# wenjundeng/pic1dp

Hardware: AMD Instinct MI355X
Metric: particle-updates/sec (higher is better)
Workload: dtype f64

## Files before the change

pic1dp_amd/csrc/kernels_step.hip:

```cpp
#include "device_diag.hpp"
#include "device_field.hpp"
#include "device_fx.hpp"
#include "device_math.hpp"
#include "device_xchg.hpp"
#include "step_args.hpp"

#include <cstdio>
#include <type_traits>
#include <vector>

#ifndef PIC1DP_STEP_DIST
#error "compile with -DPIC1DP_STEP_DIST=0..5 (pic1dp_amd/build.py does)"
#endif

namespace pic1dp {

namespace {

#ifdef PIC1DP_TUNE_STAMPS
#define STAMP(a, k)                                                                          \
  do {                                                                                       \
    if (threadIdx.x == 0) (a).stamps[static_cast<size_t>(blockIdx.x) * 8 + (k)] = wall_clock64(); \
  } while (0)
#define STAMP_HWID(a)                                                                                             \
// ... 174 lines not shown
__device__ __forceinline__ double pred_coef_core(double v, double w, double p, double dt, const SpeciesConst &s, D &dv,
                                                 double &t2) {
  const double tmp1 = (MODE == MODE_DF_LIN) ? p : (p - w);
  t2 = dlnf0<DIST, POW2>(v, s, dv);
  return divc<POW2>(dt * tmp1 * t2 * s.Z, s.m, s.r_m, dv);
}
template <int DIST, int MODE, int POW2>
__device__ __forceinline__ double pred_coef(double v, double w, double p, double dt, const SpeciesConst &s, double &t2) {
  if constexpr (POW2 == 0) {
    if (s.fastc) {
      DivFast dv;
      const double c = pred_coef_core<DIST, MODE, POW2>(v, w, p, dt, s, dv, t2);
      if (dv.ok()) return c;
    }
  }
  DivTrue dv;
  return pred_coef_core<DIST, MODE, POW2>(v, w, p, dt, s, dv, t2);
}

struct FxTiles {
  double s0, s1;
  float mx0, mx1;
};
__device__ __forceinline__ double wave_uniform(double v) {
  const long long b = __double_as_longlong(v);
  const unsigned lo = static_cast<unsigned>(__builtin_amdgcn_readfirstlane(static_cast<int>(b)));
  const unsigned hi = static_cast<unsigned>(__builtin_amdgcn_readfirstlane(static_cast<int>(b >> 32)));
  return __longlong_as_double(static_cast<long long>((static_cast<unsigned long long>(hi) << 32) | lo));
}
__device__ __forceinline__ double fx_scale(double lim, double markers) {
  const double t = lim * markers;
  return t > 0.0 && t < 0x1p900 ? ldexp(1.0, 60 - ilogb(t)) : __builtin_inf();
}
__device__ __forceinline__ void pred_add_fx(double *p, double v, double s) {
  const double t = fma(v, s, 6755399441055744.0);
  __hip_atomic_fetch_add(reinterpret_cast<unsigned long long *>(p),
                         static_cast<unsigned long long>(__double_as_longlong(t)) - 0x4338000000000000ull, __ATOMIC_RELAXED,
                         __HIP_MEMORY_SCOPE_WORKGROUP);
}
__device__ __forceinline__ void fx_note(unsigned *slot, float seen_f) {
  for (int off = 32; off > 0; off >>= 1) seen_f = fmaxf(seen_f, __shfl_down(seen_f, off, 64));
  if ((threadIdx.x & 63) == 0) {
    const unsigned code = seen_f >= 0.0f ? __float_as_uint(seen_f) + 2u : (seen_f > -1.5f ? 1u : 0u);
    __hip_atomic_fetch_max(slot, code, __ATOMIC_RELAXED, __HIP_MEMORY_SCOPE_WORKGROUP);
  }
}

template <int DIST, int MODE, int POW2, int NM>
__device__ __forceinline__ double pred_one(const One &n, double p, int ix, double wl, const double *sAB, double *sP,
                                           const StepArgsDev &a, FxTiles &fx) {
  constexpr int nm = NM, np1 = 1 + 2 * NM;
  const double xh = fma(a.dt_half, n.v, n.x);
  const double sh = xh * a.snx;
  const double fh = floor(sh);
  int ih = static_cast<int>(fh);
  const double wr = sh - fh, wh = 1.0 - wr;
  ih = ih < 0 ? ih + a.g.nx : ih;
  ih = ih > a.g.nx ? ih - a.g.nx : ih;
  if (static_cast<unsigned>(ih) > static_cast<unsigned>(a.g.nx)) {
    ih = ih % a.g.nx;
    if (ih < 0) ih += a.g.nx;
  }
  double *cl = sP + __mul24(ih, np1), *cr = cl + np1;
  double t2 = 0.0;
  auto slow = [&](int k, double vl, double vr) {
    const int nx = a.g.nx;
    const int gl_c = ih >= nx ? ih - nx : ih;
    int gr_c = ih + 1;
    gr_c = gr_c >= nx ? gr_c - nx : gr_c;
    gr_c = gr_c >= nx ? gr_c - nx : gr_c;
    if (vl != 0.0) glb_add(a.pred + static_cast<size_t>(k) * nx + gl_c, vl);
    if (vr != 0.0) glb_add(a.pred + static_cast<size_t>(k) * nx + gr_c, vr);
    if (vl != 0.0 || vr != 0.0)
      __hip_atomic_fetch_add(reinterpret_cast<unsigned long long *>(a.fxb + 2), 1ull, __ATOMIC_RELAXED, __HIP_MEMORY_SCOPE_AGENT);
  };
  if constexpr (MODE == MODE_FULLF) {
    const double aq = fabs(p);
    const bool fixed = aq * fx.s0 <= a.fx_cap;
    fx.mx0 = fmaxf(fx.mx0, (fixed || fx.s0 > 0x1p1000) ? static_cast<float>(aq) : -1.0f);
    if (fixed) {
      pred_add_fx(cl, wh * p, fx.s0);
      pred_add_fx(cr, wr * p, fx.s0);
    } else {
      slow(0, wh * p, wr * p);
    }
  } else {
    const double tmp1 = (MODE == MODE_DF_LIN) ? p : (p - n.w);
    if constexpr (POW2 == 0) {
      if (a.s.fastc) {
        DivFast dv;
        t2 = dlnf0<DIST, POW2>(n.v, a.s, dv);
        if (!dv.ok()) {
          DivTrue dt;
          t2 = dlnf0<DIST, POW2>(n.v, a.s, dt);
        }
      } else {
        DivTrue dt;
        t2 = dlnf0<DIST, POW2>(n.v, a.s, dt);
      }
    } else {
      DivTrue dt;
      t2 = dlnf0<DIST, POW2>(n.v, a.s, dt);
    }
    const double c = tmp1 * t2 * a.pred_k;
    const double aq = fabs(n.w), ac = fabs(c);
    const bool ok0 = aq * fx.s0 <= a.fx_cap, ok1 = 2.0 * ac * fx.s1 <= a.fx_cap;
    fx.mx0 = fmaxf(fx.mx0, (ok0 || fx.s0 > 0x1p1000) ? static_cast<float>(aq) : -1.0f);
    fx.mx1 = fmaxf(fx.mx1, (ok1 || fx.s1 > 0x1p1000) ? static_cast<float>(ac) : -1.0f);
    const bool fixed = ok0 && ok1;
    if (fixed) {
      pred_add_fx(cl, wh * n.w, fx.s0);
      pred_add_fx(cr, wr * n.w, fx.s0);
    } else {
      slow(0, wh * n.w, wr * n.w);
    }
    const double *gl = sAB + __mul24(ix, 2 * nm), *gr = gl + 2 * nm;
    const double wlr = 1.0 - wl;
#pragma unroll
    for (int m = 0; m < nm; ++m) {
      const double2 tl = *reinterpret_cast<const double2 *>(gl + 2 * m), tr = *reinterpret_cast<const double2 *>(gr + 2 * m);
      const double A = fma(tr.x, wlr, tl.x * wl), B = fma(tr.y, wlr, tl.y * wl);
      const double cA = c * A, cB = c * B;
      if (fixed) {
        pred_add_fx(cl + 1 + m, wh * cA, fx.s1);
        pred_add_fx(cr + 1 + m, wr * cA, fx.s1);
        pred_add_fx(cl + 1 + nm + m, wh * cB, fx.s1);
        pred_add_fx(cr + 1 + nm + m, wr * cB, fx.s1);
      } else {
        slow(1 + m, wh * cA, wr * cA);
        slow(1 + nm + m, wh * cB, wr * cB);
      }
    }
  }
  return t2;
}

constexpr int FUSED_CHAIN_W = 8;
struct TabCells {
  double *ab;
  __device__ __forceinline__ void put(int c, double a, double b) const { ab[2 * c] = a, ab[2 * c + 1] = b; }
  __device__ __forceinline__ void get(int c, double &a, double &b) const { a = ab[2 * c], b = ab[2 * c + 1]; }
};
struct TabTiles {
  double *sa, *sb;
  __device__ __forceinline__ void put(int c, double a, double b) const { sa[c] = a, sb[c] = b; }
  __device__ __forceinline__ void get(int c, double &a, double &b) const { a = sa[c], b = sb[c]; }
};
template <bool TILE_EH, class TAB>
__device__ __forceinline__ void fused_solve(const FusedSolve &fs, const TAB &tab, double *sE0, double *sX, double *sSc,
                                            double &re_h, double &im_h, unsigned long long *stamps = nullptr) {
  (void)stamps;
  const FieldArgs &f = fs.f;
  const int nx = f.nx;
  double *sMode = sSc, *sScr = sSc + 8, *sPart = sSc + 24;
  const bool lead = blockIdx.x == 0;
  double *sPc = sE0, *sPs = sX;
  for (int ix = threadIdx.x; ix < nx; ix += blockDim.x) {
    double c2 = 0.0;
    for (int sp = 0; sp < f.nspecies; ++sp) {
      const double *r = f.rho_sp + static_cast<size_t>(sp) * nx + ix;
      double c1 = *r;
      for (int g = 1; g < f.rho_copies; ++g) c1 = c1 + r[static_cast<size_t>(g) * f.rho_stride];
      c2 = c2 + c1 * f.Z[sp];
    }
    const double cd = chargeden_from(f, c2);
    if (lead) {
      f.charge[ix] = c2;
      f.chargeden[ix] = cd;
    }
    const double tr = f.fre[ix], ti = f.fim[ix];
    tab.put(ix, 2.0 * tr, 2.0 * ti);
    if (ix == 0) tab.put(nx, 2.0 * tr, 2.0 * ti);
    sPc[ix] = tr * cd;
    sPs[ix] = ti * cd;
  }
  if (lead) {
    for (int64_t i = threadIdx.x; i < fs.zero_rho_n; i += blockDim.x) fs.zero_rho[i] = 0.0;
    for (int i = threadIdx.x; i < 8 * PRED_SUM_COPIES; i += blockDim.x) fs.zero_pred[i] = 0.0;
  }
  __syncthreads();
  STAMP_SOLVE(stamps, 2);
  const double ginv = f.grad_inv[0];
  {
    const double acc = lean_forward_sums<FUSED_CHAIN_W>(f, sPc, sPs, sPart, [&]() {
      const int k = static_cast<int>(threadIdx.x) - (static_cast<int>(blockDim.x) - 64);
      if (k >= 0 && k < 6) {
        double a = 0.0;
        static_assert(PRED_SUM_COPIES % 8 == 0, "eight copies in flight at a time");
        for (int c0 = 0; c0 < PRED_SUM_COPIES; c0 += 8) {
          double t[8];
#pragma unroll
          for (int c = 0; c < 8; ++c) t[c] = fs.pred_in[(c0 + c) * 8 + k];
#pragma unroll
          for (int c = 0; c < 8; ++c) a = (c0 + c == 0) ? t[0] : a + t[c];
        }
        sMode[2 + k] = a;
      }
    });
    if (threadIdx.x < 2) mode_store(f, sMode, 1, 0, threadIdx.x == 0, acc, ginv, lead);
  }
  __syncthreads();
  STAMP_SOLVE(stamps, 3);
  const double re = sMode[0], im = sMode[1];
  double ac, as;
  pred_forward_sums(f, fs.pt, sMode + 2, re, im, ac, as);
  STAMP_SOLVE(stamps, 4);
  im_h = mode_scale(f, true, ac, ginv);
  re_h = mode_scale(f, false, as, ginv);
  if (lead && threadIdx.x == 0) {
    fs.mode_h[0] = re_h;
    fs.mode_h[1] = im_h;
  }
  double e2 = 0.0;
  for (int ix = threadIdx.x; ix < nx; ix += blockDim.x) {
    double tA, tB;
    tab.get(ix, tA, tB);
    const double tr = 0.5 * tA, ti = 0.5 * tB;
    const double e = inverse_one_mode(tr, ti, re, im), eh = inverse_one_mode(tr, ti, re_h, im_h);
    sE0[ix] = e;
    if constexpr (TILE_EH) sX[ix] = eh;
    if (ix == 0) {
      sE0[nx] = e;
      if constexpr (TILE_EH) sX[nx] = eh;
    }
    e2 += e * e;
    if (lead) {
      f.E[ix] = e;
      fs.E_h[ix] = eh;
    }
  }
  if (lead && f.history) field_energy_store(e2, sScr, f.lx, f.dnx, f.history);
}

constexpr int PRIV_THREADS = STEP_PRIVATE_THREADS;
template <int DIST, int MODE, int POW2>
__device__ __forceinline__ double pred_one_private(const One &n, double p, int ix, double wl, const double *sAB, double *sS,
                                                   const StepArgsDev &a) {
  constexpr int stride = PRIV_THREADS;
  const int nx = a.g.nx;
  double t2 = 0.0, cA = 0.0, cB = 0.0;
  if constexpr (MODE != MODE_FULLF) {
    const double tmp1 = (MODE == MODE_DF_LIN) ? p : (p - n.w);
    if constexpr (POW2 == 0) {
      if (a.s.fastc) {
        DivFast dv;
        t2 = dlnf0<DIST, POW2>(n.v, a.s, dv);
        if (!dv.ok()) {
          DivTrue dt;
          t2 = dlnf0<DIST, POW2>(n.v, a.s, dt);
        }
      } else {
        DivTrue dt;
        t2 = dlnf0<DIST, POW2>(n.v, a.s, dt);
      }
    } else {
      DivTrue dt;
      t2 = dlnf0<DIST, POW2>(n.v, a.s, dt);
    }
    const double c = tmp1 * t2 * (a.pred_k * a.s.Z);
    const double *gl = sAB + 2 * ix;
    const double2 tl = *reinterpret_cast<const double2 *>(gl), tr = *reinterpret_cast<const double2 *>(gl + 2);
    const double wlr = 1.0 - wl;
    cA = c * fma(tr.x, wlr, tl.x * wl);
    cB = c * fma(tr.y, wlr, tl.y * wl);
  }
  const double xh = fma(a.dt_half, n.v, n.x);
  const double sh = xh * a.snx;
  const double fh = floor(sh);
  int ih = static_cast<int>(fh);
  const double wr = sh - fh, wh = 1.0 - wr;
  ih = ih < 0 ? ih + nx : ih;
  ih = ih >= nx ? ih - nx : ih;
  if (static_cast<unsigned>(ih) >= static_cast<unsigned>(nx)) {
    ih = ih % nx;
    if (ih < 0) ih += nx;
  }
  const double *hl = sAB + 2 * ih;
  const double2 ul = *reinterpret_cast<const double2 *>(hl), ur = *reinterpret_cast<const double2 *>(hl + 2);
  const double Ah = fma(ur.x, wr, ul.x * wh), Bh = fma(ur.y, wr, ul.y * wh);
  const double q = a.s.Z * (MODE == MODE_FULLF ? p : n.w);
  lds_add(sS, q * Ah);
  lds_add(sS + 3 * stride, q * Bh);
  if constexpr (MODE != MODE_FULLF) {
    lds_add(sS + stride, cA * Ah);
    lds_add(sS + 2 * stride, cB * Ah);
    lds_add(sS + 4 * stride, cA * Bh);
    lds_add(sS + 5 * stride, cB * Bh);
  }
  return t2;
}


template <int DIST, int MODE, int POW2, int NM>
__device__ __forceinline__ double priv_sums(const One &n, double p, int ix, double wl, const double *sAB, double *sS,
                                            const StepArgsDev &a) {
  return pred_one_private<DIST, MODE, POW2>(n, p, ix, wl, sAB, sS, a);
}

template <bool NT>
__device__ __forceinline__ bool chunk_plain(int64_t j, const StepArgsDev &a) {
  if constexpr (!NT) return false;
  return __builtin_amdgcn_readfirstlane(static_cast<int>(j >> 6)) < a.plain_chunks;
}
template <bool NT, bool HAS_W>
__device__ __forceinline__ void ld_marker_rows(bool plain, const double2 *x2, const double2 *v2, const double2 *w2, const double2 *p2,
                                               int64_t o, double2 &X, double2 &V, double2 &W, double2 &P) {
  if (NT && plain) {
    X = ld2t<false>(x2 + o), V = ld2t<false>(v2 + o), P = ld2t<false>(p2 + o);
    if constexpr (HAS_W) W = ld2t<false>(w2 + o);
  } else {
    X = ld2t<NT>(x2 + o), V = ld2t<NT>(v2 + o), P = ld2t<NT>(p2 + o);
    if constexpr (HAS_W) W = ld2t<NT>(w2 + o);
  }
}
template <bool NT, bool PUSH_V, bool HAS_W>
__device__ __forceinline__ void st_marker_rows(bool plain, double2 *x2, double2 *v2, double2 *w2, int64_t o, const One &n0, const One &n1) {
  if (NT && plain) {
    st2t<false>(x2 + o, n0.x, n1.x);
    if constexpr (PUSH_V) st2t<false>(v2 + o, n0.v, n1.v);
    if constexpr (HAS_W) st2t<false>(w2 + o, n0.w, n1.w);
  } else {
    st2t<NT>(x2 + o, n0.x, n1.x);
    if constexpr (PUSH_V) st2t<NT>(v2 + o, n0.v, n1.v);
    if constexpr (HAS_W) st2t<NT>(w2 + o, n0.w, n1.w);
  }
}

template <int DIST, int MODE, int POW2, bool NT, int T2, int NM, bool PRIV = false, bool FUSED = false>
__global__ void __launch_bounds__(1024) PIC1DP_SIX_WAVES k_step_one(const StepArgsDev a) {
  static_assert(!FUSED || PRIV, "the fused solve serves the six-sum prediction");
  constexpr int NS = 6, PT = PRIV_THREADS;
  static_assert(!PRIV || NM == 1, "six sums: one kept mode");
  extern __shared__ __attribute__((aligned(16))) char smem[];
  STAMP(a, 0);
  STAMP_HWID(a);
  exp_table_init();
  const int nx = a.g.nx;
  constexpr int nm = NM, np1 = 1 + 2 * NM;
  const int ne = (nx + 2) & ~1;
  double *sE0 = reinterpret_cast<double *>(smem);
  double *sEh = sE0 + ne;
  double *sAB = sEh + ne;
  double *sR0 = sAB + static_cast<size_t>(nx + 1) * 2 * nm;
  double *sP = sR0 + ((nx + 2) & ~1);
  if constexpr (!FUSED) {
    for (int i = threadIdx.x; i < nx; i += blockDim.x) {
      sE0[i] = a.E0[i];
      sEh[i] = a.Eh[i];
    }
  }
  if constexpr (!FUSED) {
    for (int i = threadIdx.x; i < nm * (nx + 1); i += blockDim.x) {
      const int m = i / (nx + 1), c = i - m * (nx + 1), cs = c < nx ? c : 0;
      sAB[c * 2 * nm + 2 * m] = a.tabA[m * nx + cs];
      sAB[c * 2 * nm + 2 * m + 1] = a.tabB[m * nx + cs];
    }
  }
  zero_rho(sR0, a.g);
  if constexpr (FUSED) {
    double re_h, im_h;
#ifdef PIC1DP_TUNE_STAMPS
    fused_solve<true>(a.fused, TabCells{sAB}, sE0, sEh, sP, re_h, im_h, a.stamps);
#else
    fused_solve<true>(a.fused, TabCells{sAB}, sE0, sEh, sP, re_h, im_h);
#endif
    __syncthreads();
  } else if (threadIdx.x == 0) {
    sE0[nx] = a.E0[0];
    sEh[nx] = a.Eh[0];
  }
  unsigned *sDraw = reinterpret_cast<unsigned *>(PRIV ? sP + NS * PT : sP + np1 * (nx + 2));
  FxTiles fx{};
  fx.mx0 = fx.mx1 = -2.0f;
  double fxb_start0 = 0.0, fxb_start1 = 0.0;
  if constexpr (PRIV) {
    for (int k = 0; k < NS; ++k) sP[k * PT + threadIdx.x] = 0.0;
  } else {
    if (threadIdx.x == 0) {
      sP[0] = __hip_atomic_load(a.fxb, __ATOMIC_RELAXED, __HIP_MEMORY_SCOPE_AGENT);
      sP[1] = __hip_atomic_load(a.fxb + 1, __ATOMIC_RELAXED, __HIP_MEMORY_SCOPE_AGENT);
    }
    __syncthreads();
    fxb_start0 = wave_uniform(sP[0]);
    fxb_start1 = wave_uniform(sP[1]);
    fx.s0 = wave_uniform(fx_scale(16.0 * fxb_start0, a.fx_markers));
    fx.s1 = wave_uniform(fx_scale(32.0 * fxb_start1, a.fx_markers));
    __syncthreads();
    for (int i = threadIdx.x; i < np1 * (nx + 2); i += blockDim.x) sP[i] = 0.0;
  }
  if (threadIdx.x == 0) sDraw[0] = sDraw[1] = sDraw[2] = 0u;
  __syncthreads();
  STAMP(a, 1);
  double *sR = sR0;
  constexpr bool HAS_W = (MODE != MODE_FULLF);
  constexpr bool PUSH_V = (MODE != MODE_DF_LIN);
  constexpr bool CARRY_IN = (T2 == 2) && HAS_W;
  constexpr bool CARRY_OUT = (T2 != 0) && HAS_W;
  const int64_t npair = a.np >> 1;
  const int64_t stride = static_cast<int64_t>(gridDim.x) * blockDim.x;
  double2 *x2 = reinterpret_cast<double2 *>(a.x);
  double2 *v2 = reinterpret_cast<double2 *>(a.v);
  double2 *w2 = reinterpret_cast<double2 *>(a.w);
  const double2 *p2 = reinterpret_cast<const double2 *>(a.p);
  double2 *t2 = reinterpret_cast<double2 *>(a.t2);
  const int64_t first = static_cast<int64_t>(blockIdx.x) * blockDim.x;
  int dealt = first < npair ? static_cast<int>((npair - first + stride - 1) / stride) : 0;
  int drawn_total = 0;
  if (a.dyn_tail > 0) {
    const int drawn_rows = (dealt * a.dyn_tail) >> 4;
    dealt -= drawn_rows;
    drawn_total = drawn_rows * static_cast<int>(blockDim.x >> 6);
  }
  int64_t j = first + threadIdx.x;
  for (int k = 0;; ++k, j += stride) {
    if (k >= dealt) {
      int c = 0;
      if ((threadIdx.x & 63) == 0) c = static_cast<int>(__hip_atomic_fetch_add(sDraw, 1u, __ATOMIC_RELAXED, __HIP_MEMORY_SCOPE_WORKGROUP));
      c = __builtin_amdgcn_readfirstlane(c);
      if (c >= drawn_total) break;
      const int waves = static_cast<int>(blockDim.x >> 6);
      j = first + static_cast<int64_t>(dealt + c / waves) * stride + (c % waves) * 64 + (threadIdx.x & 63);
    }
    if (j >= npair) continue;
    const int64_t o = tidx2(j);
    const bool plain = chunk_plain<NT>(j, a);
    double2 X, V, P, W = make_double2(0.0, 0.0), T = make_double2(0.0, 0.0);
    ld_marker_rows<NT, HAS_W>(plain, x2, v2, w2, p2, o, X, V, W, P);
    if constexpr (CARRY_IN) T = ld2t<NT>(t2 + j);
    int i0, i1;
    double l0, l1;
    const One n0 = step_full_one<DIST, MODE, POW2, CARRY_IN>(X.x, V.x, W.x, P.x, sE0, sEh, sR, a, T.x, &i0, &l0);
    double u0, u1;
    if constexpr (PRIV)
      u0 = priv_sums<DIST, MODE, POW2, NM>(n0, P.x, i0, l0, sAB, sP + threadIdx.x, a);
    else
      u0 = pred_one<DIST, MODE, POW2, NM>(n0, P.x, i0, l0, sAB, sP, a, fx);
    PAIR_FENCE();
    const One n1 = step_full_one<DIST, MODE, POW2, CARRY_IN>(X.y, V.y, W.y, P.y, sE0, sEh, sR, a, T.y, &i1, &l1);
    if constexpr (PRIV)
      u1 = priv_sums<DIST, MODE, POW2, NM>(n1, P.y, i1, l1, sAB, sP + threadIdx.x, a);
    else
      u1 = pred_one<DIST, MODE, POW2, NM>(n1, P.y, i1, l1, sAB, sP, a, fx);
    st_marker_rows<NT, PUSH_V, HAS_W>(plain, x2, v2, w2, o, n0, n1);
    if constexpr (CARRY_OUT) st2t<NT>(t2 + j, u0, u1);
  }
  if ((a.np & 1) && blockIdx.x == 0 && threadIdx.x == 0) {
    const int64_t i = tidx(a.np - 1);
    const double w = HAS_W ? a.w[i] : 0.0, p = a.p[i];
    int ic;
    double lc;
    const One n = step_full_one<DIST, MODE, POW2, CARRY_IN>(a.x[i], a.v[i], w, p, sE0, sEh, sR, a,
                                                            CARRY_IN ? a.t2[a.np - 1] : 0.0, &ic, &lc);
    a.x[i] = n.x;
    if constexpr (PUSH_V) a.v[i] = n.v;
    if constexpr (HAS_W) a.w[i] = n.w;
    double u;
    if constexpr (PRIV)
      u = priv_sums<DIST, MODE, POW2, NM>(n, p, ic, lc, sAB, sP + threadIdx.x, a);
    else
      u = pred_one<DIST, MODE, POW2, NM>(n, p, ic, lc, sAB, sP, a, fx);
    if constexpr (CARRY_OUT) a.t2[a.np - 1] = u;
  }
  STAMP_LOOP(a, 2);
  if constexpr (!PRIV) {
    fx_note(sDraw + 1, fx.mx0);
    fx_note(sDraw + 2, fx.mx1);
  }
  __syncthreads();
  STAMP_LOOP(a, 3);
  flush_rho(sR0, a.rho, a.g);
  STAMP_LOOP(a, 4);
  if constexpr (PRIV) {
    const int wave = threadIdx.x >> 6, lane = threadIdx.x & 63;
    if (wave < 6) {
      const double *s = sP + wave * PRIV_THREADS + lane;
      double t = 0.0;
#pragma unroll
      for (int j = 0; j < PRIV_THREADS / 64; ++j) t += s[64 * j];
      for (int off = 32; off > 0; off >>= 1) t += __shfl_down(t, off, 64);
      if (lane == 0) glb_add(a.pred + (blockIdx.x % PRED_SUM_COPIES) * 8 + wave, t);
    }
    STAMP(a, 5);
    if constexpr (!FUSED)
      if (a.tail.mode) step_tail(a.tail, reinterpret_cast<double *>(smem));
    return;
  }
  if (threadIdx.x < 2 * np1) {
    const int g = threadIdx.x / np1, k = threadIdx.x - g * np1;
    const int to = (nx + g) % nx;
    if (g == 0 || to != 0 || nx > 1)
      __hip_atomic_fetch_add(reinterpret_cast<unsigned long long *>(&sP[to * np1 + k]),
                             static_cast<unsigned long long>(__double_as_longlong(sP[(nx + g) * np1 + k])), __ATOMIC_RELAXED,
                             __HIP_MEMORY_SCOPE_WORKGROUP);
  }
  __syncthreads();
  {
    const double q0 = 1.0 / fx.s0, q1 = 1.0 / fx.s1;
    const int rot = static_cast<int>((static_cast<long long>(blockIdx.x) * nx) / gridDim.x);
    for (int i = threadIdx.x; i < np1 * nx; i += blockDim.x) {
      const int k = i / nx;
      int c = i - k * nx + rot;
      if (c >= nx) c -= nx;
      const long long fixed = __double_as_longlong(sP[c * np1 + k]);
      if (fixed != 0) glb_add(&a.pred[static_cast<size_t>(k) * nx + c], static_cast<double>(fixed) * (k == 0 ? q0 : q1));
    }
  }
  if (threadIdx.x == 0) {
    fx_raise(a.fxb, sDraw[1], fxb_start0);
    fx_raise(a.fxb + 1, sDraw[2], fxb_start1);
  }
  STAMP(a, 5);
}

struct PredSums {
  double k0c = 0.0, k1c = 0.0, k2c = 0.0, k0s = 0.0, k1s = 0.0, k2s = 0.0;
};

template <int DIST, int MODE, int POW2>
__device__ __forceinline__ double pred_one_sums(const One &n, double p, int ix, double wl, const double *sA,
                                                const double *sB, PredSums &k, const StepArgsDev &a) {
  double t2 = 0.0;
  double cA = 0.0, cB = 0.0;
  if constexpr (MODE != MODE_FULLF) {
    const double c = a.s.Z * pred_coef<DIST, MODE, POW2>(n.v, n.w, p, a.dt_half, a.s, t2);
    PAIR_FENCE();
    double A = sA[ix] * wl;
    A = A + sA[ix + 1] * (1.0 - wl);
    double B = sB[ix] * wl;
    B = B + sB[ix + 1] * (1.0 - wl);
    cA = c * A, cB = c * B;
  }
  double xh = n.x + a.dt_half * n.v;
  xh = wrap(xh, a.g.lx);
  int ih;
  double wh;
  locate(xh, a.g, ih, wh);
  double Ah = sA[ih] * wh;
  Ah = Ah + sA[ih + 1] * (1.0 - wh);
  double Bh = sB[ih] * wh;
  Bh = Bh + sB[ih + 1] * (1.0 - wh);
  const double q = a.s.Z * (MODE == MODE_FULLF ? p : n.w);
  k.k0c += q * Ah;
  k.k0s += q * Bh;
  if constexpr (MODE != MODE_FULLF) {
    k.k1c += cA * Ah;
    k.k2c += cB * Ah;
    k.k1s += cA * Bh;
    k.k2s += cB * Bh;
  }
  return t2;
}

#ifdef PIC1DP_SUMS_WAVES
#define PIC1DP_SUMS_ATTR __attribute__((amdgpu_waves_per_eu(PIC1DP_SUMS_WAVES)))
#else
#define PIC1DP_SUMS_ATTR
#endif
template <int DIST, int MODE, int POW2, bool NT, int T2, bool FUSED = false>
__global__ void __launch_bounds__(1024) PIC1DP_SUMS_ATTR k_step_sums(const StepArgsDev a) {
  extern __shared__ __attribute__((aligned(16))) char smem[];
  STAMP(a, 0);
  STAMP_HWID(a);
  exp_table_init();
  const int nx = a.g.nx;
  const int ne = (nx + 2) & ~1;
  double *sE0 = reinterpret_cast<double *>(smem);
  double *sA = sE0 + ne;
  double *sB = sA + ne;
  double *sR0 = sB + ne;
  double *sScr = sR0 + ((nx + 2) & ~1);
  unsigned *sDraw = reinterpret_cast<unsigned *>(sScr);
  if constexpr (!FUSED) {
    for (int i = threadIdx.x; i < nx; i += blockDim.x) {
      sE0[i] = a.E0[i];
      sA[i] = a.tabA[i];
      sB[i] = a.tabB[i];
    }
    if (threadIdx.x == 0) {
      sE0[nx] = a.E0[0];
      sA[nx] = a.tabA[0];
      sB[nx] = a.tabB[0];
    }
  }
  double re_h, im_h;
  if constexpr (FUSED) {
    fused_solve<false>(a.fused, TabTiles{sA, sB}, sE0, sR0, sScr, re_h, im_h);
  } else {
    re_h = *a.eh_re;
    im_h = *a.eh_im;
  }
  zero_rho(sR0, a.g);
  if (threadIdx.x == 0) *sDraw = 0u;
  __syncthreads();
  STAMP(a, 1);
  const ModeField sEh{sA, sB, re_h, im_h};
  double *sR = sR0;
  constexpr bool HAS_W = (MODE != MODE_FULLF);
  constexpr bool PUSH_V = (MODE != MODE_DF_LIN);
  constexpr bool CARRY_IN = (T2 == 2) && HAS_W;
  constexpr bool CARRY_OUT = (T2 != 0) && HAS_W;
  PredSums ks;
  const int64_t npair = a.np >> 1;
  const int64_t stride = static_cast<int64_t>(gridDim.x) * blockDim.x;
  double2 *x2 = reinterpret_cast<double2 *>(a.x);
  double2 *v2 = reinterpret_cast<double2 *>(a.v);
  double2 *w2 = reinterpret_cast<double2 *>(a.w);
  const double2 *p2 = reinterpret_cast<const double2 *>(a.p);
  double2 *t2 = reinterpret_cast<double2 *>(a.t2);
  const int64_t first = static_cast<int64_t>(blockIdx.x) * blockDim.x;
  int dealt = first < npair ? static_cast<int>((npair - first + stride - 1) / stride) : 0;
  int drawn_total = 0;
  if (a.dyn_tail > 0) {
    const int drawn_rows = (dealt * a.dyn_tail) >> 4;
    dealt -= drawn_rows;
    drawn_total = drawn_rows * static_cast<int>(blockDim.x >> 6);
  }
  int64_t j = first + threadIdx.x;
  for (int k = 0;; ++k, j += stride) {
    if (k >= dealt) {
      int c = 0;
      if ((threadIdx.x & 63) == 0) c = static_cast<int>(__hip_atomic_fetch_add(sDraw, 1u, __ATOMIC_RELAXED, __HIP_MEMORY_SCOPE_WORKGROUP));
      c = __builtin_amdgcn_readfirstlane(c);
      if (c >= drawn_total) break;
      const int waves = static_cast<int>(blockDim.x >> 6);
      j = first + static_cast<int64_t>(dealt + c / waves) * stride + (c % waves) * 64 + (threadIdx.x & 63);
    }
    if (j >= npair) continue;
    const int64_t o = tidx2(j);
    const bool plain = chunk_plain<NT>(j, a);
    double2 X, V, P, W = make_double2(0.0, 0.0), T = make_double2(0.0, 0.0);
    ld_marker_rows<NT, HAS_W>(plain, x2, v2, w2, p2, o, X, V, W, P);
    if constexpr (CARRY_IN) T = ld2t<NT>(t2 + j);
    int i0, i1;
    double l0, l1;
    const One n0 = step_full_one<DIST, MODE, POW2, CARRY_IN>(X.x, V.x, W.x, P.x, sE0, sEh, sR, a, T.x, &i0, &l0);
    PAIR_FENCE();
    const double u0 = pred_one_sums<DIST, MODE, POW2>(n0, P.x, i0, l0, sA, sB, ks, a);
    PAIR_FENCE();
    const One n1 = step_full_one<DIST, MODE, POW2, CARRY_IN>(X.y, V.y, W.y, P.y, sE0, sEh, sR, a, T.y, &i1, &l1);
    PAIR_FENCE();
    const double u1 = pred_one_sums<DIST, MODE, POW2>(n1, P.y, i1, l1, sA, sB, ks, a);
    st_marker_rows<NT, PUSH_V, HAS_W>(plain, x2, v2, w2, o, n0, n1);
    if constexpr (CARRY_OUT) st2t<NT>(t2 + j, u0, u1);
  }
  if ((a.np & 1) && blockIdx.x == 0 && threadIdx.x == 0) {
    const int64_t i = tidx(a.np - 1);
    const double w = HAS_W ? a.w[i] : 0.0, p = a.p[i];
    int ic;
    double lc;
    const One n = step_full_one<DIST, MODE, POW2, CARRY_IN>(a.x[i], a.v[i], w, p, sE0, sEh, sR, a,
                                                            CARRY_IN ? a.t2[a.np - 1] : 0.0, &ic, &lc);
    a.x[i] = n.x;
    if constexpr (PUSH_V) a.v[i] = n.v;
    if constexpr (HAS_W) a.w[i] = n.w;
    const double u = pred_one_sums<DIST, MODE, POW2>(n, p, ic, lc, sA, sB, ks, a);
    if constexpr (CARRY_OUT) a.t2[a.np - 1] = u;
  }
  STAMP_LOOP(a, 2);
  __syncthreads();
  STAMP_LOOP(a, 3);
  flush_rho(sR0, a.rho, a.g);
  STAMP_LOOP(a, 4);
  const double mine[6] = {ks.k0c, ks.k1c, ks.k2c, ks.k0s, ks.k1s, ks.k2s};
  block_sum6_add(mine, sScr, a.pred + (blockIdx.x % PRED_SUM_COPIES) * 8);
  STAMP(a, 5);
  if constexpr (!FUSED)
    if (a.tail.mode) step_tail(a.tail, reinterpret_cast<double *>(smem));
}

#ifdef PIC1DP_TUNE_STAMPS
constexpr size_t kStampGrid = 16384;
struct StampState {
  unsigned long long *dev = nullptr;
  long launches = 0, at = -1;
  int blocks = 0, threads = 0;
};
StampState &stamp_state() {
  static StampState s;
  return s;
}
hipError_t stamp_hook(StepArgsDev &d, const LaunchCfg &lc, hipStream_t st) {
  StampState &s = stamp_state();
  if (!s.dev) {
    hipError_t e = hipMalloc(&s.dev, sizeof(unsigned long long) * 8 * kStampGrid);
    if (e != hipSuccess) return e;
    if (const char *a = tuning_env("PIC1DP_STAMP_AT")) s.at = std::atol(a);
  }
  if (s.launches == s.at + 1 && s.at >= 0) {
    hipError_t e = hipStreamSynchronize(st);
    if (e != hipSuccess) return e;
    std::vector<unsigned long long> h(static_cast<size_t>(8) * s.blocks);
    e = hipMemcpy(h.data(), s.dev, sizeof(unsigned long long) * h.size(), hipMemcpyDeviceToHost);
    if (e != hipSuccess) return e;
    if (const char *fn = tuning_env("PIC1DP_STAMP_FILE")) {
      if (FILE *f = std::fopen(fn, "w")) {
        std::fprintf(f, "# blocks %d threads %d\n", s.blocks, s.threads);
        for (int b = 0; b < s.blocks; ++b) {
          for (int k = 0; k < 7; ++k) std::fprintf(f, "%llu ", h[static_cast<size_t>(b) * 8 + k]);
          std::fprintf(f, "\n");
        }
        std::fclose(f);
      }
    }
  }
  s.launches++;
  s.blocks = lc.blocks;
  s.threads = lc.threads;
  d.stamps = s.dev;
  return static_cast<size_t>(lc.blocks) <= kStampGrid ? hipSuccess : hipErrorInvalidValue;
}
#endif

template <typename K>
hipError_t launch_step_kernel(K kern, const StepArgsDev &d0, const LaunchCfg &lc, hipStream_t st) {
#ifdef PIC1DP_TUNE_STAMPS
  StepArgsDev d = d0;
  if (hipError_t e = stamp_hook(d, lc, st); e != hipSuccess) return e;
#else
  const StepArgsDev &d = d0;
#endif
  return launch_kernel(kern, dim3(lc.blocks), dim3(lc.threads), lc.lds, st, d);
}

#ifdef PIC1DP_TUNING
template <int DIST>
constexpr bool kCarryBuilt = true;
template <int DIST>
constexpr bool kNoCarryBuilt = true;
#else
template <int DIST>
constexpr bool kCarryBuilt = DIST == 2 || DIST == 3;
template <int DIST>
constexpr bool kNoCarryBuilt = !(DIST == 2 || DIST == 3);
#endif

template <int DIST, class F>
hipError_t with_nt_t2(bool nt, int t2m, F &&f) {
  auto by_t2 = [&](auto NT) -> hipError_t {
    if constexpr (kCarryBuilt<DIST>) {
      if (t2m == 2) return f(NT, std::integral_constant<int, 2>{});
      if (t2m == 1) return f(NT, std::integral_constant<int, 1>{});
    }
    if (t2m != 0) return hipErrorInvalidValue;
    if constexpr (kNoCarryBuilt<DIST>) return f(NT, std::integral_constant<int, 0>{});
    return hipErrorInvalidValue;
  };
  return nt ? by_t2(std::true_type{}) : by_t2(std::false_type{});
}

static_assert(PRED_MAX_MODES == 2 || PRED_MAX_MODES == 3, "k_step_one is instantiated for one and two (three) kept modes");
static_assert(PRIV_THREADS == STEP_PRIVATE_THREADS, "slot stride of k_step_one<PRIV> = its workgroup size");

template <int DIST, int MODE, int POW2, bool CARRY = false>
hipError_t launch_step_dmp(const StepArgs &a, bool full, const LaunchCfg &lc, hipStream_t st) {
  const StepArgsDev &d = a.d;
  const bool one_pass = full && d.pred;
  const int t2m = d.t2 ? d.t2_mode : 0;
  if (one_pass && a.family == StepFamily::PrivateSums) {
    if (d.fused.on)
      return with_nt_t2<DIST>(d.nt, t2m, [&](auto NT, auto T2) {
        return launch_step_kernel(k_step_one<DIST, MODE, POW2, NT, T2, 1, true, true>, d, lc, st);
      });
    return with_nt_t2<DIST>(d.nt, t2m, [&](auto NT, auto T2) {
      return launch_step_kernel(k_step_one<DIST, MODE, POW2, NT, T2, 1, true>, d, lc, st);
    });
  }
  if (one_pass && a.family == StepFamily::Sums) {
    if (d.fused.on)
      return with_nt_t2<DIST>(d.nt, t2m, [&](auto NT, auto T2) {
        return launch_step_kernel(k_step_sums<DIST, MODE, POW2, NT, T2, true>, d, lc, st);
      });
    return with_nt_t2<DIST>(d.nt, t2m, [&](auto NT, auto T2) {
      return launch_step_kernel(k_step_sums<DIST, MODE, POW2, NT, T2>, d, lc, st);
    });
  }
  if (d.fx.acc) {
    if (d.pred || d.dist_out) return hipErrorInvalidValue;
    if (d.nt)
      return full ? launch_step_kernel(k_step_full<DIST, MODE, POW2, true, CARRY, false, false, true>, d, lc, st)
                  : launch_step_kernel(k_step_half<DIST, MODE, POW2, true, CARRY, true>, d, lc, st);
    return full ? launch_step_kernel(k_step_full<DIST, MODE, POW2, false, CARRY, false, false, true>, d, lc, st)
                : launch_step_kernel(k_step_half<DIST, MODE, POW2, false, CARRY, true>, d, lc, st);
  }
  if (one_pass) {
    auto tiles = [&](auto NM) {
      return with_nt_t2<DIST>(d.nt, t2m, [&](auto NT, auto T2) {
        return launch_step_kernel(k_step_one<DIST, MODE, POW2, NT, T2, NM>, d, lc, st);
      });
    };
    if (d.pred_nm == 1) return tiles(std::integral_constant<int, 1>{});
    if (d.pred_nm == 2) return tiles(std::integral_constant<int, 2>{});
    if constexpr (PRED_MAX_MODES >= 3)
      if (d.pred_nm == 3) return tiles(std::integral_constant<int, 3>{});
    return hipErrorInvalidValue;
  }
  if (full && d.dist_out) {
    if (d.diag_fx)
      return d.nt ? launch_step_kernel(k_step_full<DIST, MODE, POW2, true, CARRY, true, true>, d, lc, st)
                  : launch_step_kernel(k_step_full<DIST, MODE, POW2, false, CARRY, true, true>, d, lc, st);
    return d.nt ? launch_step_kernel(k_step_full<DIST, MODE, POW2, true, CARRY, true>, d, lc, st)
                : launch_step_kernel(k_step_full<DIST, MODE, POW2, false, CARRY, true>, d, lc, st);
  }
  if (d.nt)
    return full ? launch_step_kernel(k_step_full<DIST, MODE, POW2, true, CARRY, false>, d, lc, st)
                : launch_step_kernel(k_step_half<DIST, MODE, POW2, true, CARRY>, d, lc, st);
  return full ? launch_step_kernel(k_step_full<DIST, MODE, POW2, false, CARRY, false>, d, lc, st)
              : launch_step_kernel(k_step_half<DIST, MODE, POW2, false, CARRY>, d, lc, st);
}

template <int DIST>
hipError_t launch_step_d(const StepArgs &a, bool full, const LaunchCfg &lc, hipStream_t st) {
  const StepArgsDev &d = a.d;
  const bool pow2 = d.s.pow2 != 0;
  if (!a.deltaf) {
    if constexpr (DIST == 0)
      return pow2 ? launch_step_dmp<0, MODE_FULLF, 1>(a, full, lc, st)
                  : launch_step_dmp<0, MODE_FULLF, 0>(a, full, lc, st);
    return hipErrorInvalidValue;
  }
  const bool carry = !pow2 && d.t2 != nullptr && (DIST == 2 || DIST == 3);
  if (a.linear) {
    if constexpr (DIST == 2 || DIST == 3)
      if (carry) return launch_step_dmp<DIST, MODE_DF_LIN, 0, true>(a, full, lc, st);
    return pow2 ? launch_step_dmp<DIST, MODE_DF_LIN, 1>(a, full, lc, st)
                : launch_step_dmp<DIST, MODE_DF_LIN, 0>(a, full, lc, st);
  }
  if (d.s.unit) return launch_step_dmp<DIST, MODE_DF_NL, 2>(a, full, lc, st);
  if constexpr (DIST == 2 || DIST == 3)
    if (carry) return launch_step_dmp<DIST, MODE_DF_NL, 0, true>(a, full, lc, st);
  return pow2 ? launch_step_dmp<DIST, MODE_DF_NL, 1>(a, full, lc, st)
              : launch_step_dmp<DIST, MODE_DF_NL, 0>(a, full, lc, st);
}

}

template <>
hipError_t launch_step_dist<PIC1DP_STEP_DIST>(const StepArgs &a, bool full, const LaunchCfg &lc, hipStream_t st) {
  return launch_step_d<PIC1DP_STEP_DIST>(a, full, lc, st);
}

}
```

Before: 215.7 billion.

## Restructure particle loop into wave-uniform chunks with optional row prefetch

Replaces the per-thread grid-stride loop with wave-granular chunk scheduling. Chunk base addresses are computed as scalar (readfirstlane) values plus a per-lane 16-byte offset, which should reduce per-lane 64-bit address arithmetic and VGPR use. Adds an optional software prefetch of the next chunk's X/V (or all four) rows, controlled by PIC1DP_PREFETCH_ROWS. That option defaults to 0, so by default only the addressing and scheduling restructure takes effect. Prefetching would raise register pressure in exchange for hiding load latency.

After: 215.6 billion, median of 3. No clear change (-0.1%).

```diff
diff --git a/pic1dp_amd/csrc/kernels_step.hip b/pic1dp_amd/csrc/kernels_step.hip
--- a/pic1dp_amd/csrc/kernels_step.hip
+++ b/pic1dp_amd/csrc/kernels_step.hip
@@ -500,29 +500,95 @@
   if constexpr (!NT) return false;
   return __builtin_amdgcn_readfirstlane(static_cast<int>(j >> 6)) < a.plain_chunks;
 }
-template <bool NT, bool HAS_W>
-__device__ __forceinline__ void ld_marker_rows(bool plain, const double2 *x2, const double2 *v2, const double2 *w2, const double2 *p2,
-                                               int64_t o, double2 &X, double2 &V, double2 &W, double2 &P) {
+
+struct WaveChunks {
+  int64_t first, stride;
+  int wave, waves;
+  int dealt, drawn_total;
+  int k;
+};
+__device__ __forceinline__ WaveChunks wave_chunks(int64_t npair, int dyn_tail) {
+  WaveChunks w;
+  w.first = static_cast<int64_t>(blockIdx.x) * blockDim.x;
+  w.stride = static_cast<int64_t>(gridDim.x) * blockDim.x;
+  w.wave = __builtin_amdgcn_readfirstlane(static_cast<int>(threadIdx.x >> 6));
+  w.waves = static_cast<int>(blockDim.x >> 6);
+  w.dealt = w.first < npair ? static_cast<int>((npair - w.first + w.stride - 1) / w.stride) : 0;
+  w.drawn_total = 0;
+  if (dyn_tail > 0) {
+    const int drawn_rows = (w.dealt * dyn_tail) >> 4;
+    w.dealt -= drawn_rows;
+    w.drawn_total = drawn_rows * w.waves;
+  }
+  w.k = 0;
+  return w;
+}
+__device__ __forceinline__ int64_t next_chunk(WaveChunks &w, int64_t npair, unsigned *sDraw) {
+  for (;;) {
+    int64_t j0;
+    if (w.k < w.dealt) {
+      j0 = w.first + static_cast<int64_t>(w.k) * w.stride + w.wave * 64;
+      ++w.k;
+    } else {
+      int c = 0;
+      if ((threadIdx.x & 63) == 0) c = static_cast<int>(__hip_atomic_fetch_add(sDraw, 1u, __ATOMIC_RELAXED, __HIP_MEMORY_SCOPE_WORKGROUP));
+      c = __builtin_amdgcn_readfirstlane(c);
+      if (c >= w.drawn_total) return -1;
+      j0 = w.first + static_cast<int64_t>(w.dealt + c / w.waves) * w.stride + (c % w.waves) * 64;
+    }
+    if (j0 < npair) return j0;
+  }
+}
+__device__ __forceinline__ bool chunk_lane(int64_t j0, int64_t npair, unsigned lane16) {
+  const int64_t left = npair - j0;
+  return lane16 < (left < 64 ? static_cast<unsigned>(left) << 4 : 1024u);
+}
+template <class T>
+__device__ __forceinline__ T *chunk_row(T *array, int64_t ob, unsigned lane16) {
+  const unsigned long long b = reinterpret_cast<unsigned long long>(array) + static_cast<unsigned long long>(ob);
+  const unsigned lo = static_cast<unsigned>(__builtin_amdgcn_readfirstlane(static_cast<int>(b)));
+  const unsigned hi = static_cast<unsigned>(__builtin_amdgcn_readfirstlane(static_cast<int>(b >> 32)));
+  using G = __attribute__((address_space(1))) T;
+  return (T *)reinterpret_cast<G *>(((static_cast<unsigned long long>(hi) << 32) | lo) + lane16);
+}
+template <bool NT, bool HAS_W, int R0, int R1>
+__device__ __forceinline__ void ld_chunk_rows(bool plain, const StepArgsDev &a, int64_t ob, unsigned lane16, double2 &X, double2 &V,
+                                              double2 &W, double2 &P) {
+  const double2 *x2 = chunk_row(reinterpret_cast<const double2 *>(a.x), ob, lane16);
+  const double2 *v2 = chunk_row(reinterpret_cast<const double2 *>(a.v), ob, lane16);
+  const double2 *p2 = chunk_row(reinterpret_cast<const double2 *>(a.p), ob, lane16);
+  const double2 *w2 = chunk_row(reinterpret_cast<const double2 *>(a.w), ob, lane16);
   if (NT && plain) {
-    X = ld2t<false>(x2 + o), V = ld2t<false>(v2 + o), P = ld2t<false>(p2 + o);
-    if constexpr (HAS_W) W = ld2t<false>(w2 + o);
+    if constexpr (R0 <= 0 && 0 < R1) X = ld2t<false>(x2);
+    if constexpr (R0 <= 1 && 1 < R1) V = ld2t<false>(v2);
+    if constexpr (R0 <= 2 && 2 < R1) P = ld2t<false>(p2);
+    if constexpr (HAS_W && R0 <= 3 && 3 < R1) W = ld2t<false>(w2);
   } else {
-    X = ld2t<NT>(x2 + o), V = ld2t<NT>(v2 + o), P = ld2t<NT>(p2 + o);
-    if constexpr (HAS_W) W = ld2t<NT>(w2 + o);
+    if constexpr (R0 <= 0 && 0 < R1) X = ld2t<NT>(x2);
+    if constexpr (R0 <= 1 && 1 < R1) V = ld2t<NT>(v2);
+    if constexpr (R0 <= 2 && 2 < R1) P = ld2t<NT>(p2);
+    if constexpr (HAS_W && R0 <= 3 && 3 < R1) W = ld2t<NT>(w2);
   }
 }
 template <bool NT, bool PUSH_V, bool HAS_W>
-__device__ __forceinline__ void st_marker_rows(bool plain, double2 *x2, double2 *v2, double2 *w2, int64_t o, const One &n0, const One &n1) {
+__device__ __forceinline__ void st_chunk_rows(bool plain, const StepArgsDev &a, int64_t ob, unsigned lane16, const One &n0, const One &n1) {
+  double2 *x2 = chunk_row(reinterpret_cast<double2 *>(a.x), ob, lane16);
+  double2 *v2 = chunk_row(reinterpret_cast<double2 *>(a.v), ob, lane16);
+  double2 *w2 = chunk_row(reinterpret_cast<double2 *>(a.w), ob, lane16);
   if (NT && plain) {
-    st2t<false>(x2 + o, n0.x, n1.x);
-    if constexpr (PUSH_V) st2t<false>(v2 + o, n0.v, n1.v);
-    if constexpr (HAS_W) st2t<false>(w2 + o, n0.w, n1.w);
+    st2t<false>(x2, n0.x, n1.x);
+    if constexpr (PUSH_V) st2t<false>(v2, n0.v, n1.v);
+    if constexpr (HAS_W) st2t<false>(w2, n0.w, n1.w);
   } else {
-    st2t<NT>(x2 + o, n0.x, n1.x);
-    if constexpr (PUSH_V) st2t<NT>(v2 + o, n0.v, n1.v);
-    if constexpr (HAS_W) st2t<NT>(w2 + o, n0.w, n1.w);
-  }
-}
+    st2t<NT>(x2, n0.x, n1.x);
+    if constexpr (PUSH_V) st2t<NT>(v2, n0.v, n1.v);
+    if constexpr (HAS_W) st2t<NT>(w2, n0.w, n1.w);
+  }
+}
+#ifndef PIC1DP_PREFETCH_ROWS
+#define PIC1DP_PREFETCH_ROWS 0
+#endif
+static_assert(PIC1DP_PREFETCH_ROWS == 0 || PIC1DP_PREFETCH_ROWS == 2 || PIC1DP_PREFETCH_ROWS == 4, "none, X and V, or all four rows");
 
 template <int DIST, int MODE, int POW2, bool NT, int T2, int NM, bool PRIV = false, bool FUSED = false>
 __global__ void __launch_bounds__(1024) PIC1DP_SIX_WAVES k_step_one(const StepArgsDev a) {
@@ -595,52 +661,53 @@
   constexpr bool CARRY_IN = (T2 == 2) && HAS_W;
   constexpr bool CARRY_OUT = (T2 != 0) && HAS_W;
   const int64_t npair = a.np >> 1;
-  const int64_t stride = static_cast<int64_t>(gridDim.x) * blockDim.x;
-  double2 *x2 = reinterpret_cast<double2 *>(a.x);
-  double2 *v2 = reinterpret_cast<double2 *>(a.v);
-  double2 *w2 = reinterpret_cast<double2 *>(a.w);
-  const double2 *p2 = reinterpret_cast<const double2 *>(a.p);
   double2 *t2 = reinterpret_cast<double2 *>(a.t2);
-  const int64_t first = static_cast<int64_t>(blockIdx.x) * blockDim.x;
-  int dealt = first < npair ? static_cast<int>((npair - first + stride - 1) / stride) : 0;
-  int drawn_total = 0;
-  if (a.dyn_tail > 0) {
-    const int drawn_rows = (dealt * a.dyn_tail) >> 4;
-    dealt -= drawn_rows;
-    drawn_total = drawn_rows * static_cast<int>(blockDim.x >> 6);
-  }
-  int64_t j = first + threadIdx.x;
-  for (int k = 0;; ++k, j += stride) {
-    if (k >= dealt) {
-      int c = 0;
-      if ((threadIdx.x & 63) == 0) c = static_cast<int>(__hip_atomic_fetch_add(sDraw, 1u, __ATOMIC_RELAXED, __HIP_MEMORY_SCOPE_WORKGROUP));
-      c = __builtin_amdgcn_readfirstlane(c);
-      if (c >= drawn_total) break;
-      const int waves = static_cast<int>(blockDim.x >> 6);
-      j = first + static_cast<int64_t>(dealt + c / waves) * stride + (c % waves) * 64 + (threadIdx.x & 63);
-    }
-    if (j >= npair) continue;
-    const int64_t o = tidx2(j);
-    const bool plain = chunk_plain<NT>(j, a);
-    double2 X, V, P, W = make_double2(0.0, 0.0), T = make_double2(0.0, 0.0);
-    ld_marker_rows<NT, HAS_W>(plain, x2, v2, w2, p2, o, X, V, W, P);
-    if constexpr (CARRY_IN) T = ld2t<NT>(t2 + j);
-    int i0, i1;
-    double l0, l1;
-    const One n0 = step_full_one<DIST, MODE, POW2, CARRY_IN>(X.x, V.x, W.x, P.x, sE0, sEh, sR, a, T.x, &i0, &l0);
-    double u0, u1;
-    if constexpr (PRIV)
-      u0 = priv_sums<DIST, MODE, POW2, NM>(n0, P.x, i0, l0, sAB, sP + threadIdx.x, a);
-    else
-      u0 = pred_one<DIST, MODE, POW2, NM>(n0, P.x, i0, l0, sAB, sP, a, fx);
-    PAIR_FENCE();
-    const One n1 = step_full_one<DIST, MODE, POW2, CARRY_IN>(X.y, V.y, W.y, P.y, sE0, sEh, sR, a, T.y, &i1, &l1);
-    if constexpr (PRIV)
-      u1 = priv_sums<DIST, MODE, POW2, NM>(n1, P.y, i1, l1, sAB, sP + threadIdx.x, a);
-    else
-      u1 = pred_one<DIST, MODE, POW2, NM>(n1, P.y, i1, l1, sAB, sP, a, fx);
-    st_marker_rows<NT, PUSH_V, HAS_W>(plain, x2, v2, w2, o, n0, n1);
-    if constexpr (CARRY_OUT) st2t<NT>(t2 + j, u0, u1);
+  constexpr int PF = PIC1DP_PREFETCH_ROWS;
+  const unsigned lane16 = (threadIdx.x & 63u) << 4;
+  WaveChunks wc = wave_chunks(npair, a.dyn_tail);
+  double2 X = make_double2(0.0, 0.0), V = X, P = X, W = X, Xn = X, Vn = X, Pn = X, Wn = X;
+  int64_t j0 = next_chunk(wc, npair, sDraw);
+  if constexpr (PF > 0)
+    if (j0 >= 0 && chunk_lane(j0, npair, lane16))
+      ld_chunk_rows<NT, HAS_W, 0, PF>(chunk_plain<NT>(j0, a), a, tidx2(j0) << 4, lane16, Xn, Vn, Wn, Pn);
+  while (j0 >= 0) {
+    const int64_t ob = tidx2(j0) << 4;
+    const bool plain = chunk_plain<NT>(j0, a);
+    const bool mine = chunk_lane(j0, npair, lane16);
+    int64_t jn = -1;
+    double2 T = make_double2(0.0, 0.0);
+    if constexpr (PF > 0) {
+      X = Xn, V = Vn;
+      if constexpr (PF > 2) P = Pn, W = Wn;
+      jn = next_chunk(wc, npair, sDraw);
+    }
+    if (mine) {
+      ld_chunk_rows<NT, HAS_W, PF, 4>(plain, a, ob, lane16, X, V, W, P);
+      if constexpr (CARRY_IN) T = ld2t<NT>(chunk_row(t2, j0 << 4, lane16));
+    }
+    if constexpr (PF > 0)
+      if (jn >= 0 && chunk_lane(jn, npair, lane16))
+        ld_chunk_rows<NT, HAS_W, 0, PF>(chunk_plain<NT>(jn, a), a, tidx2(jn) << 4, lane16, Xn, Vn, Wn, Pn);
+    if (mine) {
+      int i0, i1;
+      double l0, l1;
+      const One n0 = step_full_one<DIST, MODE, POW2, CARRY_IN>(X.x, V.x, W.x, P.x, sE0, sEh, sR, a, T.x, &i0, &l0);
+      double u0, u1;
+      if constexpr (PRIV)
+        u0 = priv_sums<DIST, MODE, POW2, NM>(n0, P.x, i0, l0, sAB, sP + threadIdx.x, a);
+      else
+        u0 = pred_one<DIST, MODE, POW2, NM>(n0, P.x, i0, l0, sAB, sP, a, fx);
+      PAIR_FENCE();
+      const One n1 = step_full_one<DIST, MODE, POW2, CARRY_IN>(X.y, V.y, W.y, P.y, sE0, sEh, sR, a, T.y, &i1, &l1);
+      if constexpr (PRIV)
+        u1 = priv_sums<DIST, MODE, POW2, NM>(n1, P.y, i1, l1, sAB, sP + threadIdx.x, a);
+      else
+        u1 = pred_one<DIST, MODE, POW2, NM>(n1, P.y, i1, l1, sAB, sP, a, fx);
+      st_chunk_rows<NT, PUSH_V, HAS_W>(plain, a, ob, lane16, n0, n1);
+      if constexpr (CARRY_OUT) st2t<NT>(chunk_row(t2, j0 << 4, lane16), u0, u1);
+    }
+    if constexpr (PF == 0) jn = next_chunk(wc, npair, sDraw);
+    j0 = jn;
   }
   if ((a.np & 1) && blockIdx.x == 0 && threadIdx.x == 0) {
     const int64_t i = tidx(a.np - 1);
@@ -799,47 +866,48 @@
   constexpr bool CARRY_OUT = (T2 != 0) && HAS_W;
   PredSums ks;
   const int64_t npair = a.np >> 1;
-  const int64_t stride = static_cast<int64_t>(gridDim.x) * blockDim.x;
-  double2 *x2 = reinterpret_cast<double2 *>(a.x);
-  double2 *v2 = reinterpret_cast<double2 *>(a.v);
-  double2 *w2 = reinterpret_cast<double2 *>(a.w);
-  const double2 *p2 = reinterpret_cast<const double2 *>(a.p);
   double2 *t2 = reinterpret_cast<double2 *>(a.t2);
-  const int64_t first = static_cast<int64_t>(blockIdx.x) * blockDim.x;
-  int dealt = first < npair ? static_cast<int>((npair - first + stride - 1) / stride) : 0;
-  int drawn_total = 0;
-  if (a.dyn_tail > 0) {
-    const int drawn_rows = (dealt * a.dyn_tail) >> 4;
-    dealt -= drawn_rows;
-    drawn_total = drawn_rows * static_cast<int>(blockDim.x >> 6);
-  }
-  int64_t j = first + threadIdx.x;
-  for (int k = 0;; ++k, j += stride) {
-    if (k >= dealt) {
-      int c = 0;
-      if ((threadIdx.x & 63) == 0) c = static_cast<int>(__hip_atomic_fetch_add(sDraw, 1u, __ATOMIC_RELAXED, __HIP_MEMORY_SCOPE_WORKGROUP));
-      c = __builtin_amdgcn_readfirstlane(c);
-      if (c >= drawn_total) break;
-      const int waves = static_cast<int>(blockDim.x >> 6);
-      j = first + static_cast<int64_t>(dealt + c / waves) * stride + (c % waves) * 64 + (threadIdx.x & 63);
-    }
-    if (j >= npair) continue;
-    const int64_t o = tidx2(j);
-    const bool plain = chunk_plain<NT>(j, a);
-    double2 X, V, P, W = make_double2(0.0, 0.0), T = make_double2(0.0, 0.0);
-    ld_marker_rows<NT, HAS_W>(plain, x2, v2, w2, p2, o, X, V, W, P);
-    if constexpr (CARRY_IN) T = ld2t<NT>(t2 + j);
-    int i0, i1;
-    double l0, l1;
-    const One n0 = step_full_one<DIST, MODE, POW2, CARRY_IN>(X.x, V.x, W.x, P.x, sE0, sEh, sR, a, T.x, &i0, &l0);
-    PAIR_FENCE();
-    const double u0 = pred_one_sums<DIST, MODE, POW2>(n0, P.x, i0, l0, sA, sB, ks, a);
-    PAIR_FENCE();
-    const One n1 = step_full_one<DIST, MODE, POW2, CARRY_IN>(X.y, V.y, W.y, P.y, sE0, sEh, sR, a, T.y, &i1, &l1);
-    PAIR_FENCE();
-    const double u1 = pred_one_sums<DIST, MODE, POW2>(n1, P.y, i1, l1, sA, sB, ks, a);
-    st_marker_rows<NT, PUSH_V, HAS_W>(plain, x2, v2, w2, o, n0, n1);
-    if constexpr (CARRY_OUT) st2t<NT>(t2 + j, u0, u1);
+  constexpr int PF = PIC1DP_PREFETCH_ROWS;
+  const unsigned lane16 = (threadIdx.x & 63u) << 4;
+  WaveChunks wc = wave_chunks(npair, a.dyn_tail);
+  double2 X = make_double2(0.0, 0.0), V = X, P = X, W = X, Xn = X, Vn = X, Pn = X, Wn = X;
+  int64_t j0 = next_chunk(wc, npair, sDraw);
+  if constexpr (PF > 0)
+    if (j0 >= 0 && chunk_lane(j0, npair, lane16))
+      ld_chunk_rows<NT, HAS_W, 0, PF>(chunk_plain<NT>(j0, a), a, tidx2(j0) << 4, lane16, Xn, Vn, Wn, Pn);
+  while (j0 >= 0) {
+    const int64_t ob = tidx2(j0) << 4;
+    const bool plain = chunk_plain<NT>(j0, a);
+    const bool mine = chunk_lane(j0, npair, lane16);
+    int64_t jn = -1;
+    double2 T = make_double2(0.0, 0.0);
+    if constexpr (PF > 0) {
+      X = Xn, V = Vn;
+      if constexpr (PF > 2) P = Pn, W = Wn;
+      jn = next_chunk(wc, npair, sDraw);
+    }
+    if (mine) {
+      ld_chunk_rows<NT, HAS_W, PF, 4>(plain, a, ob, lane16, X, V, W, P);
+      if constexpr (CARRY_IN) T = ld2t<NT>(chunk_row(t2, j0 << 4, lane16));
+    }
+    if constexpr (PF > 0)
+      if (jn >= 0 && chunk_lane(jn, npair, lane16))
+        ld_chunk_rows<NT, HAS_W, 0, PF>(chunk_plain<NT>(jn, a), a, tidx2(jn) << 4, lane16, Xn, Vn, Wn, Pn);
+    if (mine) {
+      int i0, i1;
+      double l0, l1;
+      const One n0 = step_full_one<DIST, MODE, POW2, CARRY_IN>(X.x, V.x, W.x, P.x, sE0, sEh, sR, a, T.x, &i0, &l0);
+      PAIR_FENCE();
+      const double u0 = pred_one_sums<DIST, MODE, POW2>(n0, P.x, i0, l0, sA, sB, ks, a);
+      PAIR_FENCE();
+      const One n1 = step_full_one<DIST, MODE, POW2, CARRY_IN>(X.y, V.y, W.y, P.y, sE0, sEh, sR, a, T.y, &i1, &l1);
+      PAIR_FENCE();
+      const double u1 = pred_one_sums<DIST, MODE, POW2>(n1, P.y, i1, l1, sA, sB, ks, a);
+      st_chunk_rows<NT, PUSH_V, HAS_W>(plain, a, ob, lane16, n0, n1);
+      if constexpr (CARRY_OUT) st2t<NT>(chunk_row(t2, j0 << 4, lane16), u0, u1);
+    }
+    if constexpr (PF == 0) jn = next_chunk(wc, npair, sDraw);
+    j0 = jn;
   }
   if ((a.np & 1) && blockIdx.x == 0 && threadIdx.x == 0) {
     const int64_t i = tidx(a.np - 1);
```
